# eltoto1219/vltk

Hardware: AMD Instinct MI355X
Metric: images/sec FRCNN feature extraction, 800x1333 batch (higher is better)
Workload: dtype f16; 1 GPU; configs[1]: ResNet-101-C4 fp16 (the reference has no FPN: SURVEY.md D1), 32 synthetic 800x1333 images per GPU per step, R=300 RPN proposals through the Res5 head, max 100 detections/img, seeded synthetic weights; global_batch=32, parallelism=image-sharded x1, all-gather of output blocks

## Files before the change

### include/vltk_hip.h

```cpp
#ifndef VLTK_HIP_H
#define VLTK_HIP_H

#include <stddef.h>
#include <stdint.h>

#ifdef __cplusplus
extern "C" {
#endif

#define VK_OK 0
#define VK_EINVAL 1
#define VK_ENOTIMPL 2
#define VK_ENONFINITE 3
#define VK_EWEIGHTS 4
#define VK_EHIP 5
#define VK_ENOMEM 6

typedef enum { VK_F32 = 0, VK_F16 = 1, VK_I64 = 2, VK_I32 = 3, VK_BF16 = 4 } vk_dtype;
typedef enum { VK_ACT_NONE = 0, VK_ACT_RELU = 1, VK_ACT_GELU = 2 , VK_ACT_TANH = 3 } vk_act;

#define VK_MAX_ANCHOR_DIM 8
#define VK_MAX_NMS_THRESH 8

typedef struct vk_config {
// ... 141 lines not shown
int vk_packed_cout(int cout);
int vk_conv_slice_channels(int cin, int groups);
int vk_pack_conv_weight(const float *w_oihw_host, const float *bn_host, const float *bias_host,
                        int cout, int cin, int kh, int kw, int groups, vk_dtype dt,
                        void *w_packed_host, float *bias_packed_host);

int vk_conv2d(const void *x, int N, int H, int W, int cin,
              const void *w_packed, const float *bias_packed, const void *residual,
              void *y, int cout, int ldy, int kh, int kw, int stride, int pad, int dil, int groups,
              int relu, vk_dtype dt, vk_dtype out_dt, void *stream);

#define VK_ROUTE_GENERIC 0
#define VK_ROUTE_RING 1
#define VK_ROUTE_DUO 2
#define VK_ROUTE_WS 3
#define VK_ROUTE_GEMM4 4
#define VK_ROUTE_PANEL 5
#define VK_ROUTE_BLK 6
int vk_conv_route(int N, int H, int W, int cin, int cin2, int has_residual, int fused_mean, int cout, int ldy, int kh, int kw,
                  int stride, int pad, int dil, int groups, int relu, vk_dtype dt, vk_dtype out_dt);
int vk_panel_phase_images(int N, int H, int W, int dil);
int vk_panel_phase_tile_rows(int N, int H, int W, int dil, int cout);
int vk_panel_phase_reuse(int N, int H, int W, int dil, int cout);

int vk_conv1x1_dual(const void *x1, int cin1, const void *x2, int cin2, long M,
                    const void *w_packed, const float *bias_packed, const void *residual,
                    void *y, int cout, int relu, void *stream);

int vk_bottleneck64(const void *x, int N, int H, int W, int cin, int proj,
                    const void *w1_packed, const float *b1_packed, const void *w2_packed, const float *b2_packed,
                    const void *w3_packed, const float *b3_packed, void *y, void *stream);

int vk_fuse_shortcut(int cin, int cin_shortcut, int cout, int stride, vk_dtype dt);
int vk_bottleneck64_eligible(int cin, int cmid, int cout, int stride, int dil, int groups, int proj, int fused_shortcut,
                             long N, int H, int W, vk_dtype dt);

size_t vk_conv1x1_meanpool_workspace_bytes(int N, int HW, int cout);
int vk_conv1x1_meanpool(const void *x, int N, int HW, int cin, const void *w_packed, const float *bias_packed,
                        const void *residual, int cout, int relu, float *out_mean,
                        void *workspace, size_t workspace_bytes, void *stream);


int vk_linear(const void *x, long M, int K, const void *w_packed, const float *bias_packed, const void *residual,
              void *y, int N, int ldy, int act, vk_dtype dt, vk_dtype out_dt, void *stream);
int vk_layernorm(const void *x, int ldx, const float *gamma, const float *beta, void *y, int ldy, int M, int C,
                 float eps, float scale, int accumulate, vk_dtype dt, void *stream);
// ... 167 lines not shown
```

### vltk_amd/_lib.py

```python
import ctypes as C
import os

_HERE = os.path.dirname(os.path.abspath(__file__))
LIB_PATH = os.path.join(_HERE, "libvltk_hip.so")
if os.environ.get("VLTK_AMD_LIB"):
    LIB_PATH = os.environ["VLTK_AMD_LIB"]
elif os.environ.get("VLTK_AMD_ABLATION_LIB") == "1":
    LIB_PATH = LIB_PATH.replace("libvltk_hip.so", "libvltk_hip_ablation.so")

VK_OK, VK_EINVAL, VK_ENOTIMPL, VK_ENONFINITE, VK_EWEIGHTS, VK_EHIP, VK_ENOMEM = range(7)
VK_F32, VK_F16, VK_I64, VK_I32, VK_BF16 = 0, 1, 2, 3, 4
VK_ACT_NONE, VK_ACT_RELU, VK_ACT_GELU, VK_ACT_TANH = 0, 1, 2, 3
VK_ROUTE_GENERIC, VK_ROUTE_RING, VK_ROUTE_DUO, VK_ROUTE_WS, VK_ROUTE_GEMM4, VK_ROUTE_PANEL, VK_ROUTE_BLK = range(7)
VK_ATT_ROUTE_MFMA, VK_ATT_ROUTE_LDS, VK_ATT_ROUTE_TILED, VK_ATT_ROUTE_STREAM = range(4)
VK_CE_FORM_VEC, VK_CE_FORM_SCALAR = 0, 1
VK_RA_FORM_SEP, VK_RA_FORM_VEC, VK_RA_FORM_SCALAR = 0, 1, 2
VK_MAX_ANCHOR_DIM = 8
VK_MAX_NMS_THRESH = 8
VK_MAX_IGNOREY = 64
VK_SELECT_CLASS_MAX, VK_SELECT_PER_CLASS, VK_SELECT_DETECTIONS = 0, 1, 2
VK_POOLER_ROIPOOL, VK_POOLER_ROIALIGN, VK_POOLER_ROIALIGNV2 = 0, 1, 2

_EXC = {
    VK_EINVAL: ValueError,
# ... 71 lines not shown
                                      C.POINTER(C.c_int64), C.POINTER(vk_ignorey)]),
    "vk_forward_begin_select": (_I, [_P, _P, _I, _I, _I, _P, _P, C.POINTER(vk_select_params), C.POINTER(vk_outputs), _P,
                                     C.POINTER(C.c_int64), C.POINTER(vk_ignorey)]),
    "vk_forward_boxes_begin": (_I, [_P, _P, _I, _I, _I, _P, _P, _P, _I, _P, C.POINTER(vk_outputs), _P, C.POINTER(C.c_int64)]),
    "vk_forward_grid_begin": (_I, [_P, _P, _I, _I, _I, _P, _P, _I, _I, C.POINTER(vk_outputs), _P, C.POINTER(C.c_int64)]),
    "vk_grid_pool": (_I, [_P, _I, _I, _I, _I, _I, _P, _P, _I, _I, _I, _P, _I, _P, _P]),
    "vk_forward_end": (_I, [_P, C.c_int64]),
    "vk_given_boxes_ingest": (_I, [_P, _P, _P, _P, _I, _I, _P, _P, _P, _I, _I, _F, _I, _P, _P]),
    "vk_given_box_outputs": (_I, [_P, _P, _P, _P, _P, _P, _P, _P, _I, _I, _I, C.POINTER(vk_outputs), _P]),
    "vk_get_stage": (_I, [_P, C.c_char_p, C.POINTER(_P), C.POINTER(_I), C.POINTER(C.c_int64), C.POINTER(_I)]),
    "vk_memcpy_d2d": (_I, [_P, _P, _SZ, _P]),
    "vk_enable_stage_timing": (_I, [_P, _I]),
    "vk_get_stage_timing": (_I, [_P, C.POINTER(_F)]),
    "vk_enable_kernel_timing": (_I, [_P, _I]),
    "vk_get_kernel_timing": (_I, [_P, C.POINTER(C.c_int64), C.POINTER(_D), C.POINTER(_D), C.POINTER(_D), _I]),
    "vk_packed_weight_bytes": (_SZ, [_I, _I, _I, _I, _I, _I]),
    "vk_conv_slice_channels": (_I, [_I, _I]),
    "vk_packed_cout": (_I, [_I]),
    "vk_pack_conv_weight": (_I, [_P, _P, _P, _I, _I, _I, _I, _I, _I, _P, _P]),
    "vk_conv_route": (_I, [_I] * 18),
    "vk_panel_phase_images": (_I, [_I, _I, _I, _I]),
    "vk_panel_phase_tile_rows": (_I, [_I, _I, _I, _I, _I]),
    "vk_panel_phase_reuse": (_I, [_I, _I, _I, _I, _I]),
    "vk_conv1x1_dual": (_I, [_P, _I, _P, _I, C.c_long, _P, _P, _P, _P, _I, _I, _P]),
    "vk_bottleneck64": (_I, [_P, _I, _I, _I, _I, _I, _P, _P, _P, _P, _P, _P, _P, _P]),
    "vk_fuse_shortcut": (_I, [_I, _I, _I, _I, _I]),
    "vk_bottleneck64_eligible": (_I, [_I, _I, _I, _I, _I, _I, _I, _I, C.c_long, _I, _I, _I]),
    "vk_conv1x1_meanpool_workspace_bytes": (_SZ, [_I, _I, _I]),
    "vk_conv1x1_meanpool": (_I, [_P, _I, _I, _I, _P, _P, _P, _I, _I, _P, _P, _SZ, _P]),
    "vk_linear": (_I, [_P, C.c_long, _I, _P, _P, _P, _P, _I, _I, _I, _I, _I, _P]),
    "vk_layernorm": (_I, [_P, _I, _P, _P, _P, _I, _I, _I, _F, _F, _I, _I, _P]),
    "vk_embed_layernorm": (_I, [_P, _P, _I, _I, _P, _P, _P, _P, _P, _P, _I, _F, _I, _P]),
    "vk_attention": (_I, [_P, _I, _P, _I, _P, _I, _P, _P, _I, _I, _I, _I, _I, _I, _I, _P]),
    "vk_attention_tiled": (_I, [_P, _I, _P, _I, _P, _I, _P, _P, _I, _I, _I, _I, _I, _I, _I, _P]),
    "vk_attention_route": (_I, [_I] * 9),
    "vk_visualbert_embed": (_I, [_P, _P, _P, _P, _I, _I, _I, _I, _P, _I, _P, _I, _P, _P, _I, _P, _P, _I, _P, _P, _P, _I, _F, _I, _P]),
    "vk_vit_patchify": (_I, [_P, _I, _I, _I, _I, _I, _P, _I, _I, _P]),
    "vk_vit_assemble": (_I, [_P, _I, _P, _P, _I, _I, _P, _I, _I, _P]),
    "vk_layoutlm_embed": (_I, [_P, _P, _P, _I, _I, _P, _I, _P, _I, _P, _P, _P, _P, _I, _P, _I, _P, _P, _P, _I, _F, _I, _P]),
    "vk_token_word_labels": (_I, [_P, _I, _P, _I, _I, _I, _I, _P, _P, _I, _P]),
    "vk_span_select": (_I, [_P, _I, _P, _I, _P, _I, _I, _I, _P, _P, _P, _I, _P]),
    "vk_cross_entropy": (_I, [_P, _I, _I, _I, _P, _I, _P, _I, _P]),
    "vk_cross_entropy_form": (_I, [_I, _I, _I, _I]),
    "vk_smooth_l1_rows": (_I, [_P, _I, _P, _I, _I, _I, _P, _I, _P]),
    "vk_loss_reduce": (_I, [_P, _P, _P, _I, _I, _F, _P, _P]),
    "vk_loss_total": (_I, [_P, _I, _P, _P]),
# ... 78 lines not shown
```

### vltk_amd/csrc/conv3x3_panel.hip

```cpp
#include <cstdio>
#include <type_traits>
#include <vector>

#include "vk_common.h"

namespace vk {

typedef _Float16 half8 __attribute__((ext_vector_type(8)));
typedef float floatx4 __attribute__((ext_vector_type(4)));
typedef _Float16 half4 __attribute__((ext_vector_type(4)));
typedef unsigned uintx4 __attribute__((ext_vector_type(4)));

struct PanelK {
    const char *x;
    const char *w;
    const float *bias;
    const char *res;
    char *y;
    int H, W, HW, M;
    int cin_bytes, ldy;
    int dil;
    int cstages;
    int wrow_bytes;
    int relu;
// ... 57 lines not shown
    static_assert(N >= 0 && N <= 15, "vmcnt immediate");
    asm volatile("s_waitcnt vmcnt(%0)" ::"n"(N) : "memory");
}

constexpr int P_WIN = 10;
constexpr int reuse_slot(int dx, int mi) { return mi + dx + 1; }
constexpr int reuse_tile(int dy, int slot, int w2) { return dy * w2 + slot - 1; }
constexpr int reuse_read_dx(int slot) { return slot < 8 ? -1 : slot - 8; }
constexpr bool reuse_window_ok() {
    for (int w2 = 1; w2 <= 7; ++w2)
        for (int dy = -1; dy <= 1; ++dy)
            for (int dx = -1; dx <= 1; ++dx)
                for (int mi = 0; mi < 8; ++mi) {
                    const int s = reuse_slot(dx, mi);
                    if (s < 0 || s >= P_WIN) return false;
                    if (reuse_tile(dy, s, w2) != mi + dy * w2 + dx) return false;
                    if (reuse_read_dx(s) > dx) return false;
                    if (reuse_tile(dy, s, w2) < -8 || reuse_tile(dy, s, w2) > 15) return false;
                }
    return true;
}
static_assert(reuse_window_ok(), "REUSE: (tap, row tile) -> window slot -> panel tile, W / 2 = 1 .. 7, inside tiles b - 8 .. b + 15");

template <int PP, int DBG, int TAG = 0, int MI = 8, int PHASE = 0, int WR = 2, int REUSE = 0>
__global__ __launch_bounds__(512, 2) void conv3x3_panel_kernel(PanelK p) {
    extern __shared__ __attribute__((aligned(16))) char smem[];
    static_assert(MI == 8 || MI == 9, "8 or 9 row tiles per wave");
    static_assert(WR == 2 || WR == 4, "2 x 4 or 4 x 2 waves");
    static_assert(!PHASE || (PP == (WR == 4 ? 6 : 4) && MI == 8 && !(DBG & 9)), "the phase form: halo 128 = (W / 2 + 1) * 16 at W = 14, 256- or 512-row tiles");
    static_assert(WR == 2 || PHASE == 2, "512 x 128 tiles: the phase form only (a plain res4 launch would read its panel twice)");
    static_assert(MI == 8 || !(DBG & 8), "the LDS-staged epilogue is written for 128-row halves");
    static_assert(!REUSE || (PHASE == 2 && WR == 4 && MI == 8 && DBG == 0), "the fragment window: tap shifts of whole 16-row tiles, 512 x 128 tiles");
    constexpr int WC = 8 / WR;
    constexpr int CT = 64 * WC;
    constexpr int NWP = CT / 128;
    constexpr int WSLOT = CT * 64;
    constexpr int TILE = WR * MI * 16;
    constexpr int PROWS = PP * 128;
    constexpr int HALO = (PROWS - TILE) / 2;
    constexpr int PBYTES = PROWS * 64;
    constexpr int WBASE = 2 * PBYTES;
    static_assert(!REUSE || (HALO / 16 == 8 && HALO / 16 + (WR - 1) * MI + 15 < PROWS / 16), "REUSE: the halo (8 tiles) covers tiles b - 8 .. b + 15");
    static_assert(HALO >= (PHASE ? 128 : 48) && WBASE + P_NW * WSLOT + (PP == 3 || WR == 4 ? 256 : 0) <= 160 * 1024, "halo / LDS");
    constexpr bool ZROW = PP == 3;
    constexpr int ZOFF = WBASE + P_NW * WSLOT;

    int bid = blockIdx.x;
    const int nwg = p.m_tiles * p.n_tiles;
    unsigned long st_k0 = 0;
    if constexpr (DBG & 4) asm volatile("s_memrealtime %0\n\ts_waitcnt lgkmcnt(0)" : "=s"(st_k0)::"memory");
    if constexpr (PP == 3 || PHASE) {
        if (p.tile_ctr && bid >= p.static_tiles) {
            constexpr bool MAIL_IN_PANEL = PHASE && WR == 2;
            int *mail = reinterpret_cast<int *>(smem + (MAIL_IN_PANEL ? 0 : ZOFF + 128));
            if (threadIdx.x == 0) {
                const unsigned v = atomicAdd(p.tile_ctr, 1u);
                if (v == p.ctr_last) *p.tile_ctr = 0u;
                *mail = p.static_tiles + (int)v;
            }
            __syncthreads();
            bid = __builtin_amdgcn_readfirstlane(*mail);
            if constexpr (MAIL_IN_PANEL) __syncthreads();
            if (bid >= nwg) return;
        }
    }
    const int q = nwg >> 3, r = nwg & 7, xcd = bid & 7;
    const int t_ = (xcd < r ? xcd * (q + 1) : r * (q + 1) + (xcd - r) * q) + (bid >> 3);
    const int n_tile = t_ % p.n_tiles, m_tile = t_ / p.n_tiles;
    const int m0 = m_tile * TILE, n0 = n_tile * CT;

    const int tid = threadIdx.x, lane = tid & 63;
    const int wave = __builtin_amdgcn_readfirstlane(tid >> 6);
    const int wr = wave / WC, wc = wave & (WC - 1);
    const int g = lane >> 4, j = lane & 15;

    unsigned vm0 = 0, vm1 = 0, vm2 = 0;

    const int lrow = lane >> 2;
    const int lchunk = (lane & 3) ^ ((-(lrow >> 2)) & 3);
    const int pm_first = m0 - HALO + wave * 16 + lrow;
    const unsigned wsrc0 = (unsigned)(n0 + wave * (16 * NWP) + lrow) * (unsigned)p.wrow_bytes + lchunk * 16;
    const unsigned wstep = 16u * p.wrow_bytes;
    int g0 = 0, gb0 = 0;
    if constexpr (PHASE) {
        g0 = (m0 >> 4) / p.HW;
        gb0 = (m0 >> 4) - g0 * p.HW;
    }
    auto blk_of = [&](int off, int &G) -> int {
        int t = gb0 + off;
        G = g0;
        while (t < 0) {
            t += p.HW;
            --G;
        }
        while (t >= p.HW) {
            t -= p.HW;
            ++G;
        }
        if (G < 0) G = 0, t = 0;
        if (G >= p.groups) G = p.groups - 1, t = p.HW - 1;
        return t;
    };
    [[maybe_unused]] unsigned ps_lane = 0, ps_blk[PP] = {};
    if constexpr (PHASE) {
        ps_lane = (unsigned)(lrow * p.HW) * (unsigned)p.cin_bytes + lchunk * 16;
#pragma unroll
        for (int q2 = 0; q2 < PP; ++q2) {
            int G;
            const int t = blk_of(wave - HALO / 16 + q2 * 8, G);
            ps_blk[q2] = __builtin_amdgcn_readfirstlane((unsigned)(G * 16 * p.HW + phase_blk(p, t).row) * (unsigned)p.cin_bytes);
        }
    }
    auto req_panel = [&](int cs, int piece) {
        if constexpr (PHASE) {
            unsigned pl = ps_lane;
            asm volatile("" : "+v"(pl));
            VKP_GLDS16(p.x + (pl + (ps_blk[piece] + cs * 64)), smem + (cs & 1) * PBYTES + (piece * 8 + wave) * 1024);
            return;
        }
        int pf = pm_first;
        asm volatile("" : "+v"(pf));
        const int m = min(max(pf + piece * 128, 0), p.M - 1);
        const unsigned off = (unsigned)m * (unsigned)p.cin_bytes + cs * 64 + lchunk * 16;
        VKP_GLDS16(p.x + off, smem + (cs & 1) * PBYTES + (piece * 8 + wave) * 1024);
    };
    auto req_w = [&](int slot, int cs, int tap, int i) {
        const unsigned koff = (unsigned)(tap * p.cstages + cs) * 64;
        unsigned wb_ = wsrc0;
        asm volatile("" : "+v"(wb_));
        VKP_GLDS16(p.w + (wb_ + i * wstep + koff), smem + WBASE + slot * WSLOT + (wave * NWP + i) * 1024);
    };

    const unsigned lds0 = (unsigned)(unsigned long)(__attribute__((address_space(3))) char *)smem;
    [[maybe_unused]] const unsigned zrow = lds0 + ZOFF;
// ... 177 lines not shown
        if constexpr (ahead) VKP_DSRX(xw[2], xa_next, 2048, twn, JN, 2);
        VKP_SB();
        VKP_MMA_ROW(7, xw[X7], wcur, tm);
        VKP_SB();
        if constexpr (MI == 9) {
            VKP_MMA_ROW(8, xw[MI == 9 ? 4 : 3], wcur, tm);
            VKP_SB();
        }
    };
    auto wset = [&](auto u_c) -> half8(&)[4] {
        if constexpr (decltype(u_c)::value % 2 == 0)
            return wa;
        else
            return wb;
    };
#define VKP_IC(V) std::integral_constant<int, (V)> {}
#define VKP_UNIT(LP, LC, U)                                                                                          \
    post(LP, VKP_IC(((U) - 1) / 9), VKP_IC(((U) - 1) % 9), cs + ((U) - 1) / 9, xan, wset(VKP_IC((U) - 1)), wset(VKP_IC(U)));  \
    xa = xan;                                                                                                        \
    pre(LC, VKP_IC((U) / 9), VKP_IC((U) % 9), xa, xan, wset(VKP_IC(U)), F_{});
    using T_ = std::integral_constant<bool, true>;
    using F_ = std::integral_constant<bool, false>;

#pragma unroll
    for (int q2 = 0; q2 < PP; ++q2) req_panel(0, q2);
#pragma unroll
    for (int st = 0; st < P_NW; ++st) {
        req_w(st, 0, st, 0);
        if constexpr (NWP == 2) req_w(st, 0, st, 1);
    }
    if constexpr (PHASE) {
        unsigned u0 = 0, u1 = 0, u2 = 0;
#pragma unroll
        for (int mi = 0; mi < MI; ++mi) {
            int G;
            const PhaseBlk b = phase_blk(p, blk_of(wr * MI + mi, G));
            const unsigned c0 = b.qx >= 1, c2 = b.qx + 1 < (p.W >> 1);
            const unsigned cw = m0 + (wr * MI + mi) * 16 < p.M ? (c0 << mi) | (1u << (9 + mi)) | (c2 << (18 + mi)) : 0u;
            u0 |= b.qy >= 1 ? cw : 0u;
            u1 |= cw;
            u2 |= b.qy + 1 < (p.H >> 1) ? cw : 0u;
        }
        vm0 = __builtin_amdgcn_readfirstlane(u0);
        vm1 = __builtin_amdgcn_readfirstlane(u1);
        vm2 = __builtin_amdgcn_readfirstlane(u2);
    } else if (p.HW >= MI * 16 + p.W) {
        const int mbase = m0 + wr * (MI * 16);
        const int rem0 = mbase % p.HW, ho0 = rem0 / p.W, wo0 = rem0 - ho0 * p.W;
        const float rcpw = 1.0f / (float)p.W;
#pragma unroll
        for (int mi = 0; mi < MI; ++mi) {
            const int xcol = wo0 + mi * 16 + j;
            int q = (int)((float)xcol * rcpw), wo = xcol - q * p.W;
            if (wo >= p.W) {
                wo -= p.W;
                ++q;
            }
            if (wo < 0) {
                wo += p.W;
                --q;
            }
            int ho = ho0 + q;
            if (ho >= p.H) ho -= p.H;
            const unsigned c0 = (unsigned)(wo - p.dil) < (unsigned)p.W, c1 = 1u, c2 = (unsigned)(wo + p.dil) < (unsigned)p.W;
            const unsigned cw = mbase + mi * 16 + j < p.M ? (c0 << mi) | (c1 << (9 + mi)) | (c2 << (18 + mi)) : 0u;
            vm0 |= (unsigned)(ho - p.dil) < (unsigned)p.H ? cw : 0u;
            vm1 |= cw;
            vm2 |= (unsigned)(ho + p.dil) < (unsigned)p.H ? cw : 0u;
// ... 1 lines not shown
    } else {
#pragma unroll
        for (int mi = 0; mi < MI; ++mi) {
            const int m = m0 + wr * (MI * 16) + mi * 16 + j;
            if (m < p.M) {
                const int n_img = m / p.HW;
                const int rem = m - n_img * p.HW;
                const int ho = rem / p.W, wo = rem - ho * p.W;
#pragma unroll
                for (int tap = 0; tap < 9; ++tap) {
                    const int hi = ho + (tap / 3 - 1) * p.dil, wi = wo + (tap % 3 - 1) * p.dil;
                    const unsigned ok = ((unsigned)hi < (unsigned)p.H && (unsigned)wi < (unsigned)p.W) ? 1u : 0u;
                    if (tap < 3)
                        vm0 |= ok << (tap * 9 + mi);
                    else if (tap < 6)
                        vm1 |= ok << ((tap - 3) * 9 + mi);
                    else
                        vm2 |= ok << ((tap - 6) * 9 + mi);
                }
            }
        }
    }

    vm_wait<NWP * (P_NW - 1)>();
    asm volatile("s_barrier" ::: "memory");
    unsigned long st_c0 = 0, st_r0 = 0;
    if constexpr (DBG & 4) asm volatile("s_memtime %0\n\ts_memrealtime %1\n\ts_waitcnt lgkmcnt(0)" : "=s"(st_c0), "=s"(st_r0)::"memory");
    unsigned xa = x_addr_of(0, 0), xan = 0;
    VKP_READ_W(wa, 0u);
    {
        [[maybe_unused]] const unsigned tw0 = tap_word(VKP_IC(0));
        VKP_DSRX(xw[0], xa, 0, tw0, 0, 0);
        VKP_DSRX(xw[1], xa, 1024, tw0, 0, 1);
        VKP_DSRX(xw[2], xa, 2048, tw0, 0, 2);
    }
    pre(F_{}, VKP_IC(0), VKP_IC(0), xa, xan, wa, T_{});
    int cs = 0;
    for (; cs + 2 < CS; cs += 2) {
        VKP_UNIT(F_{}, F_{}, 1) VKP_UNIT(F_{}, F_{}, 2) VKP_UNIT(F_{}, F_{}, 3) VKP_UNIT(F_{}, F_{}, 4) VKP_UNIT(F_{}, F_{}, 5)
        VKP_UNIT(F_{}, F_{}, 6) VKP_UNIT(F_{}, F_{}, 7) VKP_UNIT(F_{}, F_{}, 8) VKP_UNIT(F_{}, F_{}, 9) VKP_UNIT(F_{}, F_{}, 10)
        VKP_UNIT(F_{}, F_{}, 11) VKP_UNIT(F_{}, F_{}, 12) VKP_UNIT(F_{}, F_{}, 13) VKP_UNIT(F_{}, F_{}, 14) VKP_UNIT(F_{}, F_{}, 15)
        VKP_UNIT(F_{}, F_{}, 16) VKP_UNIT(F_{}, F_{}, 17)
        post(F_{}, VKP_IC(1), VKP_IC(8), cs + 1, xan, wb, wa);
        xa = xan;
        pre(F_{}, VKP_IC(0), VKP_IC(0), xa, xan, wa, F_{});
    }
    VKP_UNIT(F_{}, F_{}, 1) VKP_UNIT(F_{}, F_{}, 2) VKP_UNIT(F_{}, F_{}, 3) VKP_UNIT(F_{}, F_{}, 4) VKP_UNIT(F_{}, F_{}, 5)
    VKP_UNIT(F_{}, F_{}, 6) VKP_UNIT(F_{}, F_{}, 7) VKP_UNIT(F_{}, F_{}, 8) VKP_UNIT(F_{}, T_{}, 9) VKP_UNIT(T_{}, T_{}, 10)
    VKP_UNIT(T_{}, T_{}, 11) VKP_UNIT(T_{}, T_{}, 12) VKP_UNIT(T_{}, T_{}, 13) VKP_UNIT(T_{}, T_{}, 14) VKP_UNIT(T_{}, T_{}, 15)
    VKP_UNIT(T_{}, T_{}, 16) VKP_UNIT(T_{}, T_{}, 17)
    {
        const unsigned tm = ZROW ? 0u : tap_mask(VKP_IC(8));
        VKP_MMA_ROW(5, xw[REUSE ? reuse_slot(1, 5) : 1], wb, tm);
        VKP_MMA_ROW(6, xw[REUSE ? reuse_slot(1, 6) : 2], wb, tm);
        VKP_MMA_ROW(7, xw[REUSE ? reuse_slot(1, 7) : 3], wb, tm);
        if constexpr (MI == 9) VKP_MMA_ROW(8, xw[MI == 9 ? 4 : 3], wb, tm);
    }
    unsigned long st_c1 = 0, st_r1 = 0;
    if constexpr (DBG & 4) asm volatile("s_memtime %0\n\ts_memrealtime %1\n\ts_waitcnt lgkmcnt(0)" : "=s"(st_c1), "=s"(st_r1)::"memory");
#undef VKP_UNIT
#undef VKP_IC
#undef VKP_DSR
#undef VKP_DSRX
#undef VKP_WAIT3
#undef VKP_WAIT4
#undef VKP_MMA_ROW
#undef VKP_READ_W
#undef VKP_SB

    if constexpr (!(DBG & 8)) {
        if constexpr (PHASE) asm volatile("" : "+s"(g0), "+s"(gb0));
        auto epilogue = [&](auto res_c, auto relu_c, auto full_c) {
            constexpr bool RES = decltype(res_c)::value, RELU = decltype(relu_c)::value, FULL = decltype(full_c)::value;
            const int ch0 = n0 + wc * 64 + g * 8;
            floatx4 bq[2][2];
#pragma unroll
            for (int qn = 0; qn < 2; ++qn) {
                bq[qn][0] = *reinterpret_cast<const floatx4 *>(p.bias + ch0 + qn * 32);
                bq[qn][1] = *reinterpret_cast<const floatx4 *>(p.bias + ch0 + qn * 32 + 4);
            }
#pragma unroll
            for (int mi = 0; mi < MI; ++mi) {
                const long m = m0 + wr * (MI * 16) + mi * 16 + j;
                long mo = m;
                if constexpr (PHASE) {
                    int G;
                    const int t = blk_of(wr * MI + mi, G);
                    mo = (long)(G * 16 + j) * p.HW + phase_blk(p, t).row;
                }
                half8 rr[2];
                if constexpr (RES) {
                    const long mr = min(mo, (long)p.M - 1);
#pragma unroll
                    for (int qn = 0; qn < 2; ++qn) rr[qn] = *reinterpret_cast<const half8 *>(p.res + (mr * p.ldy + ch0 + qn * 32) * 2);
                }
#pragma unroll
                for (int qn = 0; qn < 2; ++qn) {
                    floatx4 x0 = acc[mi][2 * qn] + bq[qn][0], x1 = acc[mi][2 * qn + 1] + bq[qn][1];
                    if constexpr (RES) {
                        x0 += __builtin_convertvector(__builtin_shufflevector(rr[qn], rr[qn], 0, 1, 2, 3), floatx4);
                        x1 += __builtin_convertvector(__builtin_shufflevector(rr[qn], rr[qn], 4, 5, 6, 7), floatx4);
                    }
// ... 66 lines not shown
                if (p.relu) {
                    a = a > 0.f ? a : 0.f;
                    b = b > 0.f ? b : 0.f;
                }
                o[e] = (_Float16)a;
                o[4 + e] = (_Float16)b;
            }
            if (m < p.M) *reinterpret_cast<half8 *>(p.y + ((long)m * p.ldy + n0 + k8 * 8) * 2) = o;
        }
    };
#define VKP_LDS_BARRIER() asm volatile("s_waitcnt lgkmcnt(0)\n\ts_barrier" ::: "memory")
    half8 r0[8];
    load_res(0, r0);
    stage_half(0);
    VKP_LDS_BARRIER();
    write_half(0, r0);
    load_res(1, r0);
    VKP_LDS_BARRIER();
    stage_half(1);
    VKP_LDS_BARRIER();
    write_half(1, r0);
#undef VKP_LDS_BARRIER
    }
    if constexpr (DBG & 4) {
        unsigned long st_k1;
        asm volatile("s_waitcnt vmcnt(0)\n\ts_memrealtime %0\n\ts_waitcnt lgkmcnt(0)" : "=s"(st_k1)::"memory");
        if (threadIdx.x == 0) {
            unsigned long *o = p.stamps + (long)blockIdx.x * 6;
            o[0] = st_c1 - st_c0;
            o[1] = st_r1 - st_r0;
            o[2] = st_k1 - st_k0;
            o[3] = st_r0 - st_k0;
            o[4] = st_k0;
            o[5] = st_k1;
        }
    }
}

static int panel_pp(const ConvArgs &a, int mi = 8) {
    const int reach = a.dil * (a.W + 1);
    if (mi == 9) return reach <= 48 ? 3 : (reach <= 112 ? 4 : 0);
    return reach <= 64 ? 3 : (reach <= 128 ? 4 : 0);
}

static int panel_mi(const ConvArgs &a, long M, int n_cu) {
    if (panel_pp(a, 9) == 0) return 8;
// ... 13 lines not shown
    if ((long)a.N * a.H * a.W * a.Cin * 2 >= (1L << 32)) return false;
    return true;
}

static bool panel_phase_off() { return env_off("VK_PANEL_PHASE"); }
#ifdef VK_ABLATION
static bool panel_phase_ablation() { return env_first("VK_PANEL_PHASE") == 'A'; }
#endif

int conv3x3_panel_phase_images(const ConvArgs &a) {
    if (panel_phase_off()) return 0;
    if (a.dil != 2 || a.H % 2 != 0 || a.W % 2 != 0 || a.W > 14 || a.H > 1024 || a.N < 16) return 0;
    return a.N / 16 * 16;
}

int conv3x3_panel_phase_tile_rows(const ConvArgs &a) {
    if (a.Cout % 256 != 0 || conv3x3_panel_phase_images(a) == 0) return 0;
    return env_off("VK_PANEL_TALL") ? 256 : 512;
}

int conv3x3_panel_phase_reuse(const ConvArgs &a) {
    if (conv3x3_panel_phase_tile_rows(a) != 512) return 0;
    return env_off("VK_PANEL_REUSE") ? 0 : 1;
}

static int launch_panel_one(const ConvArgs &a, hipStream_t stream, bool phase);

int launch_conv3x3_panel(const ConvArgs &a, hipStream_t stream) {
    const int np = conv3x3_panel_phase_images(a);
    if (np == 0) return launch_panel_one(a, stream, false);
    ConvArgs b = a;
    b.N = np;
    VK_TRY(launch_panel_one(b, stream, true));
    if (np == a.N) return VK_OK;
    const size_t rows = (size_t)np * a.H * a.W;
    b.N = a.N - np;
    b.x = (const char *)a.x + rows * a.Cin * 2;
    b.y = (char *)a.y + rows * a.ldy * 2;
    if (a.res) b.res = (const char *)a.res + rows * a.ldy * 2;
    return launch_panel_one(b, stream, false);
}

static int launch_panel_one(const ConvArgs &a, hipStream_t stream, bool phase) {
    DeviceState *ds = nullptr;
    VK_TRY(device_state(&ds));
    PanelK k;
// ... 12 lines not shown
    k.M = (int)M;
    k.cin_bytes = a.Cin * 2;
    k.ldy = a.ldy;
    k.dil = a.dil;
    k.cstages = a.Cin / 32;
    k.wrow_bytes = 9 * a.Cin * 2;
    k.relu = a.relu;
    bool tall = phase && conv3x3_panel_phase_tile_rows(a) == 512;
#ifdef VK_ABLATION
    if (panel_phase_ablation()) tall = false;
#endif
    const int mi = phase ? 8 : panel_mi(a, M, ds->n_cu), pp = tall ? 6 : (phase ? 4 : panel_pp(a, mi));
    const int wslot = tall ? P_WSLOT / 2 : P_WSLOT;
    k.groups = phase ? a.N / 16 : 0;
    k.rcp_w2 = phase ? 65536u / (unsigned)(a.W / 2) + 1u : 0u;
    k.m_tiles = ceil_div(k.M, tall ? 512 : mi * 32);
    k.n_tiles = a.Cout / (tall ? 128 : 256);
    Timed t;
    VK_TRY(t.begin(stream));
    const int total_tiles = k.m_tiles * k.n_tiles;
    k.tile_ctr = nullptr;
    k.static_tiles = total_tiles;
    int n_wgs = total_tiles;
    if (!env_off("VK_PANEL_DYNAMIC") && (pp == 3 || phase) && total_tiles >= 16 * 256) {
        VK_TRY(acquire_tile_counter(&k.tile_ctr));
        k.static_tiles = total_tiles * 15 / 16 / 8 * 8;
        n_wgs = total_tiles + (total_tiles / 32 + 63) / 64 * 64;
        k.ctr_last = (unsigned)(n_wgs - k.static_tiles - 1);
    }
    const dim3 grid(n_wgs), block(512);
#ifdef VK_ABLATION
    const int dbg = env_int("VK_CONV256_DBG", 0);
#endif
    const int smem = 2 * pp * 128 * 64 + P_NW * wslot + (pp == 3 || tall ? 256 : 0);
    k.stamps = nullptr;
#define VKP_LAUNCH(PP_, DBG_, TAG_, MI_)                                                                   \
    VK_TRY(launch_lds(conv3x3_panel_kernel<PP_, DBG_, TAG_, MI_>, grid, block, smem,                       \
                      2 * PP_ * 128 * 64 + P_NW * P_WSLOT + (PP_ == 3 ? 256 : 0), stream, k))
#define VKP_LAUNCH_PHASE(...) VK_TRY(launch_lds(conv3x3_panel_kernel<__VA_ARGS__>, grid, block, smem, smem, stream, k))
#ifdef VK_ABLATION
    if (const char *sf = env_text("VK_PANEL_STAMPS"); sf && pp == 3) {
        Stamps st;
        VK_TRY(st.open((size_t)grid.x * 6, stream));
        k.stamps = st.dev;
        if (mi == 9)
            VKP_LAUNCH(3, 4, 0, 9);
        else
            VKP_LAUNCH(3, 4, 0, 8);
        VK_TRY(st.finish(stream, sf, "# wg k_loop_cycles k_loop_ticks workgroup_ticks ticks_before_k_loop start_tick end_tick (tick = 10 ns)",
                         grid.x, 6, 6, 0));
    } else if (mi == 8 && pp == 3 && dbg == 8)
        VKP_LAUNCH(3, 8, 0, 8);
    else if (mi == 8 && pp == 3 && dbg == 1)
        VKP_LAUNCH(3, 1, 0, 8);
    else if (mi == 9 && pp == 3 && dbg == 1)
        VKP_LAUNCH(3, 1, 0, 9);
    else if (mi == 9 && pp == 3 && dbg == 16)
        VKP_LAUNCH(3, 16, 0, 9);
    else if (mi == 9 && pp == 3 && dbg == 32)
        VKP_LAUNCH(3, 32, 0, 9);
    else if (phase && panel_phase_ablation())
        VKP_LAUNCH_PHASE(4, 0, 0, 8, 1);
    else
#endif
    if (tall && conv3x3_panel_phase_reuse(a))
        VKP_LAUNCH_PHASE(6, 0, 0, 8, 2, 4, 1);
    else if (tall)
        VKP_LAUNCH_PHASE(6, 0, 0, 8, 2, 4);
    else if (phase)
        VKP_LAUNCH_PHASE(4, 0, 0, 8, 2);
    else if (mi == 8 && pp == 3 && a.concurrent)
        VKP_LAUNCH(3, 0, 1, 8);
    else if (mi == 8 && pp == 3)
        VKP_LAUNCH(3, 0, 0, 8);
    else if (mi == 8 && a.concurrent)
        VKP_LAUNCH(4, 0, 1, 8);
    else if (mi == 8)
        VKP_LAUNCH(4, 0, 0, 8);
    else if (pp == 3 && a.concurrent)
        VKP_LAUNCH(3, 0, 1, 9);
    else if (pp == 3)
        VKP_LAUNCH(3, 0, 0, 9);
    else if (a.concurrent)
        VKP_LAUNCH(4, 0, 1, 9);
    else
        VKP_LAUNCH(4, 0, 0, 9);
#undef VKP_LAUNCH_PHASE
#undef VKP_LAUNCH
// ... 6 lines not shown
```

### vltk_amd/csrc/stage_api.hip

```cpp
#include <algorithm>
#include <cmath>
#include <cstdlib>

#include "vk_common.h"

using namespace vk;

namespace vk {

void fill_conv_args(ConvArgs &a, int N, int H, int W, int cin, int cout, int ldy, int k, int stride, int pad, int dil, int groups,
                    int relu, vk_dtype dt, vk_dtype out_dt) {
    memset(&a, 0, sizeof(a));
    a.N = N;
    a.H = H;
    a.W = W;
    a.Cin = cin;
    conv_out_hw(H, W, k, stride, pad, dil, &a.Ho, &a.Wo);
    a.Cout = cout;
    a.ldy = ldy;
    a.kh = a.kw = k;
    a.stride = stride;
    a.pad = pad;
    a.dil = dil;
    a.groups = groups;
// ... 173 lines not shown
    a.Cin2 = cin2;
    a.pool_part = fused_mean ? (float *)&here : nullptr;
    return conv_route_checked(a);
}

int vk_panel_phase_images(int N, int H, int W, int dil) {
    ConvArgs a;
    fill_conv_args(a, N, H, W, 128, 256, 256, 3, 1, dil, dil, 1, 0, VK_F16, VK_F16);
    return conv3x3_panel_phase_images(a);
}

int vk_panel_phase_tile_rows(int N, int H, int W, int dil, int cout) {
    ConvArgs a;
    fill_conv_args(a, N, H, W, 128, cout, cout, 3, 1, dil, dil, 1, 0, VK_F16, VK_F16);
    return conv3x3_panel_phase_tile_rows(a);
}

int vk_panel_phase_reuse(int N, int H, int W, int dil, int cout) {
    ConvArgs a;
    fill_conv_args(a, N, H, W, 128, cout, cout, 3, 1, dil, dil, 1, 0, VK_F16, VK_F16);
    return conv3x3_panel_phase_reuse(a);
}

int vk_conv1x1_dual(const void *x1, int cin1, const void *x2, int cin2, long M, const void *w_packed, const float *bias_packed,
                    const void *residual, void *y, int cout, int relu, void *stream) {
    VK_REQUIRE(x1 && x2 && M > 0 && M < (1L << 31), VK_EINVAL, "conv1x1_dual: bad arguments");
    ConvArgs a;
    fill_conv_args(a, 1, 1, (int)M, cin1, cout, cout, 1, 1, 0, 1, 1, relu, VK_F16, VK_F16);
    a.x = x1;
    a.x2 = x2;
    a.Cin2 = cin2;
    a.w = w_packed;
    a.bias = bias_packed;
    a.res = residual;
    a.y = y;
    return launch_conv(a, (hipStream_t)stream);
}

int vk_conv1x1_rows(const void *x1, int cin1, const void *x2, int cin2, long M, const int32_t *m_dev, const int32_t *x2_idx,
                    const void *w_packed, const float *bias_packed, void *y, int cout, int relu, void *stream) {
    VK_REQUIRE(x1 && w_packed && bias_packed && y && M > 0 && M < (1L << 31), VK_EINVAL, "conv1x1_rows: bad arguments");
    VK_REQUIRE(!x2_idx || x2, VK_EINVAL, "conv1x1_rows: a row index needs a second input");
    ConvArgs a;
    fill_conv_args(a, 1, 1, (int)M, cin1, cout, cout, 1, 1, 0, 1, 1, relu, VK_F16, VK_F16);
    a.x = x1;
    a.x2 = x2;
// ... 241 lines not shown
```

### vltk_amd/csrc/vk_common.h

```cpp
#pragma once
#include <hip/hip_runtime.h>

#include <atomic>
#include <cstdarg>
#include <cstdint>
#include <cstdio>
#include <cstring>
#include <vector>

#include "vltk_hip.h"

namespace vk {

void set_error(const char *fmt, ...);

#define VK_CHECK_HIP(expr)                                                                    \
    do {                                                                                      \
        hipError_t _e = (expr);                                                               \
        if (_e != hipSuccess) {                                                               \
            vk::set_error("%s:%d: %s -> %s", __FILE__, __LINE__, #expr, hipGetErrorString(_e)); \
            return VK_EHIP;                                                                   \
        }                                                                                     \
    } while (0)

// ... 49 lines not shown
    int Ho, Wo, Cout, ldy;
    int kh, kw, stride, pad, dil;
    int groups;
    int concurrent;
    float *pool_part;
    const void *x2;
    int Cin2;
    int relu;
    int stem;
    const int32_t *m_dev;
    const int32_t *x2_idx;
    vk_dtype dt, out_dt;
};
int launch_conv(const ConvArgs &a, hipStream_t stream);
int conv_route(const ConvArgs &a);
int conv_route_checked(const ConvArgs &a);
bool conv256_eligible(const ConvArgs &a);
int launch_conv256(const ConvArgs &a, hipStream_t stream);
bool conv3x3_panel_eligible(const ConvArgs &a);
int launch_conv3x3_panel(const ConvArgs &a, hipStream_t stream);
int conv3x3_panel_phase_images(const ConvArgs &a);
int conv3x3_panel_phase_tile_rows(const ConvArgs &a);
int conv3x3_panel_phase_reuse(const ConvArgs &a);
bool conv_gemm4_eligible(const ConvArgs &a);
int launch_conv_gemm4(const ConvArgs &a, hipStream_t stream);
int acquire_tile_counter(unsigned **ctr);
bool conv256_dual_ok(const ConvArgs &a);
bool conv_duo_eligible(const ConvArgs &a);
int launch_conv_duo(const ConvArgs &a, hipStream_t stream);
bool conv_ws_eligible(const ConvArgs &a);
int launch_conv_ws(const ConvArgs &a, hipStream_t stream);
bool conv3x3_blk_eligible(const ConvArgs &a);
int launch_conv3x3_blk(const ConvArgs &a, hipStream_t stream);
bool bneck_fused_eligible(int cin, int cmid, int cout, int stride, int groups, bool proj, long N, int H, int W, vk_dtype dt);
bool bneck_fused_forced();
int launch_bneck_fused(const void *x, int N, int H, int W, int cin, bool proj, const void *w1, const float *b1, const void *w2,
                       const float *b2, const void *w3, const float *b3, void *y, bool concurrent, hipStream_t stream);
bool conv_duo_dual_ok(const ConvArgs &a);
bool conv_duo_pool_ok(const ConvArgs &a);
size_t conv_duo_pool_part_bytes(long M, int Cout);
bool conv_pool_sums_f64(long N, int HW, int Cin, int Cout, bool dual);
bool conv_ws_pool_ok(const ConvArgs &a);
int launch_pool_finish(const float *part, int N, int HoWo, int Cin, int Cout, bool dual, float *out, hipStream_t stream);

struct KernelTimer {
    struct Rec {
// ... 233 lines not shown
```

Measured before the change: 542.5 images/sec.

## Make the 512x128 phase panel conv kernel persistent with next-tile prefetch

```diff
diff --git a/include/vltk_hip.h b/include/vltk_hip.h
--- a/include/vltk_hip.h
+++ b/include/vltk_hip.h
@@ -187,6 +187,7 @@
 int vk_panel_phase_images(int N, int H, int W, int dil);
 int vk_panel_phase_tile_rows(int N, int H, int W, int dil, int cout);
 int vk_panel_phase_reuse(int N, int H, int W, int dil, int cout);
+int vk_panel_persist_grid(int N, int H, int W, int dil, int cout, int n_cu);
 
 int vk_conv1x1_dual(const void *x1, int cin1, const void *x2, int cin2, long M,
                     const void *w_packed, const float *bias_packed, const void *residual,
diff --git a/vltk_amd/_lib.py b/vltk_amd/_lib.py
--- a/vltk_amd/_lib.py
+++ b/vltk_amd/_lib.py
@@ -117,6 +117,7 @@
     "vk_panel_phase_images": (_I, [_I, _I, _I, _I]),
     "vk_panel_phase_tile_rows": (_I, [_I, _I, _I, _I, _I]),
     "vk_panel_phase_reuse": (_I, [_I, _I, _I, _I, _I]),
+    "vk_panel_persist_grid": (_I, [_I, _I, _I, _I, _I, _I]),
     "vk_conv1x1_dual": (_I, [_P, _I, _P, _I, C.c_long, _P, _P, _P, _P, _I, _I, _P]),
     "vk_bottleneck64": (_I, [_P, _I, _I, _I, _I, _I, _P, _P, _P, _P, _P, _P, _P, _P]),
     "vk_fuse_shortcut": (_I, [_I, _I, _I, _I, _I]),
diff --git a/vltk_amd/csrc/conv3x3_panel.hip b/vltk_amd/csrc/conv3x3_panel.hip
--- a/vltk_amd/csrc/conv3x3_panel.hip
+++ b/vltk_amd/csrc/conv3x3_panel.hip
@@ -103,7 +103,7 @@
 }
 static_assert(reuse_window_ok(), "REUSE: (tap, row tile) -> window slot -> panel tile, W / 2 = 1 .. 7, inside tiles b - 8 .. b + 15");
 
-template <int PP, int DBG, int TAG = 0, int MI = 8, int PHASE = 0, int WR = 2, int REUSE = 0>
+template <int PP, int DBG, int TAG = 0, int MI = 8, int PHASE = 0, int WR = 2, int REUSE = 0, int PERSIST = 0>
 __global__ __launch_bounds__(512, 2) void conv3x3_panel_kernel(PanelK p) {
     extern __shared__ __attribute__((aligned(16))) char smem[];
     static_assert(MI == 8 || MI == 9, "8 or 9 row tiles per wave");
@@ -112,6 +112,8 @@
     static_assert(WR == 2 || PHASE == 2, "512 x 128 tiles: the phase form only (a plain res4 launch would read its panel twice)");
     static_assert(MI == 8 || !(DBG & 8), "the LDS-staged epilogue is written for 128-row halves");
     static_assert(!REUSE || (PHASE == 2 && WR == 4 && MI == 8 && DBG == 0), "the fragment window: tap shifts of whole 16-row tiles, 512 x 128 tiles");
+    static_assert(!PERSIST || (REUSE == 1 && PP == 6), "the tile loop: the 512 x 128 fragment-window instantiation only");
+    static_assert(!PERSIST || 1 + 4 + PP + P_NW * (64 * (8 / WR) / 128) + 2 * MI + 2 * MI <= 63, "PERSIST: a wave's outstanding vector-memory operations against vmcnt's six bits");
     constexpr int WC = 8 / WR;
     constexpr int CT = 64 * WC;
     constexpr int NWP = CT / 128;
@@ -130,7 +132,7 @@
     const int nwg = p.m_tiles * p.n_tiles;
     unsigned long st_k0 = 0;
     if constexpr (DBG & 4) asm volatile("s_memrealtime %0\n\ts_waitcnt lgkmcnt(0)" : "=s"(st_k0)::"memory");
-    if constexpr (PP == 3 || PHASE) {
+    if constexpr ((PP == 3 || PHASE) && !PERSIST) {
         if (p.tile_ctr && bid >= p.static_tiles) {
             constexpr bool MAIL_IN_PANEL = PHASE && WR == 2;
             int *mail = reinterpret_cast<int *>(smem + (MAIL_IN_PANEL ? 0 : ZOFF + 128));
@@ -145,10 +147,15 @@
             if (bid >= nwg) return;
         }
     }
-    const int q = nwg >> 3, r = nwg & 7, xcd = bid & 7;
-    const int t_ = (xcd < r ? xcd * (q + 1) : r * (q + 1) + (xcd - r) * q) + (bid >> 3);
-    const int n_tile = t_ % p.n_tiles, m_tile = t_ / p.n_tiles;
-    const int m0 = m_tile * TILE, n0 = n_tile * CT;
+    auto tile_origin = [&](int b, int &m0_, int &n0_) {
+        const int q = nwg >> 3, r = nwg & 7, xcd = b & 7;
+        const int t_ = (xcd < r ? xcd * (q + 1) : r * (q + 1) + (xcd - r) * q) + (b >> 3);
+        const int n_tile = t_ % p.n_tiles, m_tile = t_ / p.n_tiles;
+        m0_ = m_tile * TILE;
+        n0_ = n_tile * CT;
+    };
+    int m0, n0;
+    tile_origin(bid, m0, n0);
 
     const int tid = threadIdx.x, lane = tid & 63;
     const int wave = __builtin_amdgcn_readfirstlane(tid >> 6);
@@ -160,16 +167,18 @@
     const int lrow = lane >> 2;
     const int lchunk = (lane & 3) ^ ((-(lrow >> 2)) & 3);
     const int pm_first = m0 - HALO + wave * 16 + lrow;
-    const unsigned wsrc0 = (unsigned)(n0 + wave * (16 * NWP) + lrow) * (unsigned)p.wrow_bytes + lchunk * 16;
+    auto wsrc_of = [&](int n0_) -> unsigned { return (unsigned)(n0_ + wave * (16 * NWP) + lrow) * (unsigned)p.wrow_bytes + lchunk * 16; };
+    unsigned wsrc0 = wsrc_of(n0);
     const unsigned wstep = 16u * p.wrow_bytes;
     int g0 = 0, gb0 = 0;
-    if constexpr (PHASE) {
-        g0 = (m0 >> 4) / p.HW;
-        gb0 = (m0 >> 4) - g0 * p.HW;
-    }
-    auto blk_of = [&](int off, int &G) -> int {
-        int t = gb0 + off;
-        G = g0;
+    auto group_of = [&](int m0_, int &g0_, int &gb0_) {
+        g0_ = (m0_ >> 4) / p.HW;
+        gb0_ = (m0_ >> 4) - g0_ * p.HW;
+    };
+    if constexpr (PHASE) group_of(m0, g0, gb0);
+    auto blk_at = [&](int g0_, int gb0_, int off, int &G) -> int {
+        int t = gb0_ + off;
+        G = g0_;
         while (t < 0) {
             t += p.HW;
             --G;
@@ -182,15 +191,19 @@
         if (G >= p.groups) G = p.groups - 1, t = p.HW - 1;
         return t;
     };
+    auto blk_of = [&](int off, int &G) -> int { return blk_at(g0, gb0, off, G); };
     [[maybe_unused]] unsigned ps_lane = 0, ps_blk[PP] = {};
+    auto panel_src = [&](int g0_, int gb0_) {
+#pragma unroll
+        for (int q2 = 0; q2 < PP; ++q2) {
+            int G;
+            const int t = blk_at(g0_, gb0_, wave - HALO / 16 + q2 * 8, G);
+            ps_blk[q2] = __builtin_amdgcn_readfirstlane((unsigned)(G * 16 * p.HW + phase_blk(p, t).row) * (unsigned)p.cin_bytes);
+        }
+    };
     if constexpr (PHASE) {
         ps_lane = (unsigned)(lrow * p.HW) * (unsigned)p.cin_bytes + lchunk * 16;
-#pragma unroll
-        for (int q2 = 0; q2 < PP; ++q2) {
-            int G;
-            const int t = blk_of(wave - HALO / 16 + q2 * 8, G);
-            ps_blk[q2] = __builtin_amdgcn_readfirstlane((unsigned)(G * 16 * p.HW + phase_blk(p, t).row) * (unsigned)p.cin_bytes);
-        }
+        panel_src(g0, gb0);
     }
     auto req_panel = [&](int cs, int piece) {
         if constexpr (PHASE) {
@@ -414,14 +427,17 @@
     using T_ = std::integral_constant<bool, true>;
     using F_ = std::integral_constant<bool, false>;
 
-#pragma unroll
-    for (int q2 = 0; q2 < PP; ++q2) req_panel(0, q2);
-#pragma unroll
-    for (int st = 0; st < P_NW; ++st) {
-        req_w(st, 0, st, 0);
-        if constexpr (NWP == 2) req_w(st, 0, st, 1);
-    }
-    if constexpr (PHASE) {
+    auto req_prologue = [&]() {
+#pragma unroll
+        for (int q2 = 0; q2 < PP; ++q2) req_panel(0, q2);
+#pragma unroll
+        for (int st = 0; st < P_NW; ++st) {
+            req_w(st, 0, st, 0);
+            if constexpr (NWP == 2) req_w(st, 0, st, 1);
+        }
+    };
+    req_prologue();
+    auto phase_validity = [&]() {
         unsigned u0 = 0, u1 = 0, u2 = 0;
 #pragma unroll
         for (int mi = 0; mi < MI; ++mi) {
@@ -436,6 +452,9 @@
         vm0 = __builtin_amdgcn_readfirstlane(u0);
         vm1 = __builtin_amdgcn_readfirstlane(u1);
         vm2 = __builtin_amdgcn_readfirstlane(u2);
+    };
+    if constexpr (PHASE) {
+        phase_validity();
     } else if (p.HW >= MI * 16 + p.W) {
         const int mbase = m0 + wr * (MI * 16);
         const int rem0 = mbase % p.HW, ho0 = rem0 / p.W, wo0 = rem0 - ho0 * p.W;
@@ -483,10 +502,27 @@
         }
     }
 
+    unsigned long st_c0 = 0, st_r0 = 0, st_c1 = 0, st_r1 = 0;
+    typedef volatile __attribute__((address_space(3))) int *lds_word;
+    [[maybe_unused]] const lds_word mail = (lds_word)((__attribute__((address_space(3))) char *)smem + ZOFF + 128);
+    [[maybe_unused]] unsigned fetch = 0;
+    [[maybe_unused]] bool fetched = false;
+    [[maybe_unused]] floatx4 bq_pre[2][2];
+    for (;;) {
     vm_wait<NWP * (P_NW - 1)>();
     asm volatile("s_barrier" ::: "memory");
-    unsigned long st_c0 = 0, st_r0 = 0;
     if constexpr (DBG & 4) asm volatile("s_memtime %0\n\ts_memrealtime %1\n\ts_waitcnt lgkmcnt(0)" : "=s"(st_c0), "=s"(st_r0)::"memory");
+    if constexpr (PERSIST) {
+        if (fetched && tid == 0) {
+            if (fetch == p.ctr_last) *p.tile_ctr = 0u;
+            *mail = p.static_tiles + (int)fetch;
+        }
+#pragma unroll
+        for (int qn = 0; qn < 2; ++qn) {
+            bq_pre[qn][0] = *reinterpret_cast<const floatx4 *>(p.bias + n0 + wc * 64 + g * 8 + qn * 32);
+            bq_pre[qn][1] = *reinterpret_cast<const floatx4 *>(p.bias + n0 + wc * 64 + g * 8 + qn * 32 + 4);
+        }
+    }
     unsigned xa = x_addr_of(0, 0), xan = 0;
     VKP_READ_W(wa, 0u);
     {
@@ -517,8 +553,35 @@
         VKP_MMA_ROW(7, xw[REUSE ? reuse_slot(1, 7) : 3], wb, tm);
         if constexpr (MI == 9) VKP_MMA_ROW(8, xw[MI == 9 ? 4 : 3], wb, tm);
     }
-    unsigned long st_c1 = 0, st_r1 = 0;
     if constexpr (DBG & 4) asm volatile("s_memtime %0\n\ts_memrealtime %1\n\ts_waitcnt lgkmcnt(0)" : "=s"(st_c1), "=s"(st_r1)::"memory");
+
+    [[maybe_unused]] int nt = 0, nm0 = 0, nn0 = 0, ng0 = 0, ngb0 = 0;
+    if constexpr (PERSIST) {
+        asm volatile("s_barrier" ::: "memory");
+        asm volatile("" : "+s"(bid));
+        tile_origin(bid, m0, n0);
+        group_of(m0, g0, gb0);
+        asm volatile("" : "+v"(bq_pre[0][0]), "+v"(bq_pre[0][1]), "+v"(bq_pre[1][0]), "+v"(bq_pre[1][1]));
+        VKP_SB();
+        const int grid = (int)gridDim.x;
+        nt = bid + grid;
+        if (p.tile_ctr && nt >= p.static_tiles) nt = __builtin_amdgcn_readfirstlane(*mail);
+        fetched = false;
+        if (nt < nwg) {
+            tile_origin(nt, nm0, nn0);
+            group_of(nm0, ng0, ngb0);
+            panel_src(ng0, ngb0);
+            wsrc0 = wsrc_of(nn0);
+            VKP_SB();
+            req_prologue();
+            VKP_SB();
+            fetched = p.tile_ctr && nt + grid >= p.static_tiles;
+            unsigned lane_off = 0;
+            asm volatile("" : "+v"(lane_off));
+            if (fetched && tid == 0) fetch = atomicAdd(p.tile_ctr + lane_off, 1u);
+        }
+        VKP_SB();
+    }
 #undef VKP_UNIT
 #undef VKP_IC
 #undef VKP_DSR
@@ -537,8 +600,13 @@
             floatx4 bq[2][2];
 #pragma unroll
             for (int qn = 0; qn < 2; ++qn) {
-                bq[qn][0] = *reinterpret_cast<const floatx4 *>(p.bias + ch0 + qn * 32);
-                bq[qn][1] = *reinterpret_cast<const floatx4 *>(p.bias + ch0 + qn * 32 + 4);
+                if constexpr (PERSIST) {
+                    bq[qn][0] = bq_pre[qn][0];
+                    bq[qn][1] = bq_pre[qn][1];
+                } else {
+                    bq[qn][0] = *reinterpret_cast<const floatx4 *>(p.bias + ch0 + qn * 32);
+                    bq[qn][1] = *reinterpret_cast<const floatx4 *>(p.bias + ch0 + qn * 32 + 4);
+                }
             }
 #pragma unroll
             for (int mi = 0; mi < MI; ++mi) {
@@ -651,6 +719,19 @@
     write_half(1, r0);
 #undef VKP_LDS_BARRIER
     }
+    if constexpr (!PERSIST) break;
+    if (nt >= nwg) break;
+    bid = nt;
+    m0 = nm0;
+    n0 = nn0;
+    g0 = ng0;
+    gb0 = ngb0;
+    phase_validity();
+#pragma unroll
+    for (int mi = 0; mi < MI; ++mi)
+#pragma unroll
+        for (int ni = 0; ni < 4; ++ni) acc[mi][ni] = floatx4{0.f, 0.f, 0.f, 0.f};
+    }
     if constexpr (DBG & 4) {
         unsigned long st_k1;
         asm volatile("s_waitcnt vmcnt(0)\n\ts_memrealtime %0\n\ts_waitcnt lgkmcnt(0)" : "=s"(st_k1)::"memory");
@@ -710,6 +791,23 @@
 int conv3x3_panel_phase_reuse(const ConvArgs &a) {
     if (conv3x3_panel_phase_tile_rows(a) != 512) return 0;
     return env_off("VK_PANEL_REUSE") ? 0 : 1;
+}
+
+static bool panel_persist_on() {
+    const char c = env_first("VK_PANEL_PERSIST");
+    return c != '0';
+}
+int conv3x3_panel_persist_grid(const ConvArgs &a, int n_cu) {
+    if (conv3x3_panel_phase_reuse(a) == 0 || !panel_persist_on()) return 0;
+    if (n_cu <= 0) {
+        DeviceState *ds = nullptr;
+        if (const int s = device_state(&ds); s != VK_OK) return -s;
+        n_cu = ds->n_cu;
+    }
+    const long tiles = ((long)conv3x3_panel_phase_images(a) * a.H * a.W + 511) / 512 * (a.Cout / 128);
+    long grid = n_cu > 8 ? n_cu / 8 * 8 : 8;
+    if (const int cap = env_int("VK_PANEL_GRID", 0); cap > 0 && cap < grid) grid = cap;
+    return (int)(tiles < grid ? tiles : grid);
 }
 
 static int launch_panel_one(const ConvArgs &a, hipStream_t stream, bool phase);
@@ -768,6 +866,19 @@
     k.tile_ctr = nullptr;
     k.static_tiles = total_tiles;
     int n_wgs = total_tiles;
+    int persist = 0;
+    if (tall) {
+        persist = conv3x3_panel_persist_grid(a, ds->n_cu);
+        VK_REQUIRE(persist >= 0 && persist <= total_tiles, VK_EINVAL, "conv3x3_panel: persistent grid %d for %d tiles", persist, total_tiles);
+    }
+    if (persist) {
+        n_wgs = persist;
+        if (!env_off("VK_PANEL_DYNAMIC") && total_tiles >= 16 * n_wgs) {
+            VK_TRY(acquire_tile_counter(&k.tile_ctr));
+            k.static_tiles = total_tiles / n_wgs * 15 / 16 * n_wgs;
+            k.ctr_last = (unsigned)(total_tiles - k.static_tiles + n_wgs - 1);
+        }
+    } else
     if (!env_off("VK_PANEL_DYNAMIC") && (pp == 3 || phase) && total_tiles >= 16 * 256) {
         VK_TRY(acquire_tile_counter(&k.tile_ctr));
         k.static_tiles = total_tiles * 15 / 16 / 8 * 8;
@@ -809,7 +920,9 @@
         VKP_LAUNCH_PHASE(4, 0, 0, 8, 1);
     else
 #endif
-    if (tall && conv3x3_panel_phase_reuse(a))
+    if (persist)
+        VKP_LAUNCH_PHASE(6, 0, 0, 8, 2, 4, 1, 1);
+    else if (tall && conv3x3_panel_phase_reuse(a))
         VKP_LAUNCH_PHASE(6, 0, 0, 8, 2, 4, 1);
     else if (tall)
         VKP_LAUNCH_PHASE(6, 0, 0, 8, 2, 4);
diff --git a/vltk_amd/csrc/stage_api.hip b/vltk_amd/csrc/stage_api.hip
--- a/vltk_amd/csrc/stage_api.hip
+++ b/vltk_amd/csrc/stage_api.hip
@@ -219,6 +219,12 @@
     return conv3x3_panel_phase_reuse(a);
 }
 
+int vk_panel_persist_grid(int N, int H, int W, int dil, int cout, int n_cu) {
+    ConvArgs a;
+    fill_conv_args(a, N, H, W, 128, cout, cout, 3, 1, dil, dil, 1, 0, VK_F16, VK_F16);
+    return conv3x3_panel_persist_grid(a, n_cu);
+}
+
 int vk_conv1x1_dual(const void *x1, int cin1, const void *x2, int cin2, long M, const void *w_packed, const float *bias_packed,
                     const void *residual, void *y, int cout, int relu, void *stream) {
     VK_REQUIRE(x1 && x2 && M > 0 && M < (1L << 31), VK_EINVAL, "conv1x1_dual: bad arguments");
diff --git a/vltk_amd/csrc/vk_common.h b/vltk_amd/csrc/vk_common.h
--- a/vltk_amd/csrc/vk_common.h
+++ b/vltk_amd/csrc/vk_common.h
@@ -95,6 +95,7 @@
 int conv3x3_panel_phase_images(const ConvArgs &a);
 int conv3x3_panel_phase_tile_rows(const ConvArgs &a);
 int conv3x3_panel_phase_reuse(const ConvArgs &a);
+int conv3x3_panel_persist_grid(const ConvArgs &a, int n_cu);
 bool conv_gemm4_eligible(const ConvArgs &a);
 int launch_conv_gemm4(const ConvArgs &a, hipStream_t stream);
 int acquire_tile_counter(unsigned **ctr);
```

Result: no change. 545.4 images/sec, median of 6 (+0.5%).
